# hebench/reference-seal-backend

Hardware: AMD Instinct MI355X
Metric: ciphertext-ops/sec (CKKS ct x ct mul+relin+rescale, N=2^15, L=16) (higher is better)
Workload: dtype u64 (exact residues; fp64-FMA engine for primes < 2^47, u64 Harvey engine with the fold reduction for the 60-bit primes)

## Files before the change

### reference-seal-backend_amd/csrc/device_tables.h

```cpp
#pragma once
#include <cstring>
#include <vector>

#include "he_params.h"
#include "client/multiword.h"

namespace he355 {

inline void prime_dev_fill(PrimeDev &d, const PrimeTables &pt, size_t N)
{
    const ArU64 au = pt.aru();
    const ArF64 af = pt.arf();
    d.q = pt.q; d.cr0 = pt.mod.cr0; d.cr1 = pt.mod.cr1;
    d.ninv = au.ninv; d.ninv_q = au.ninv_q;
    d.qd = af.q; d.qinv = af.qinv; d.ninv_d = af.ninv; d.ninv_i = af.ninv_i;
    d.fwd = nullptr; d.inv = nullptr; d.inv_w0_scaled = pt.inv_w0_scaled;
    d.f64 = pt.f64 ? 1 : 0;
    d.acc_terms = pt.f64 ? floor_direct_terms(pt.q) : 0;
    for (size_t k = 0; k < 64; ++k) d.colw[k] = 0.0;
    if (pt.f64)
        for (size_t k = 0; k < 32 && k < N; ++k) { d.colw[k] = ArF64::tw_w(pt.fwd[k]); d.colw[32 + k] = ArF64::tw_w(pt.inv[k]); }
    d.k2_direct = d.k2_lift = 0;
    d.pow32 = (double)((((u64)1) << 32) % pt.q);
}

enum K2Class { kK2General = 0, kK2Direct = 1, kK2Lift = 2 };
inline K2Class k2_lift_class(u64 qj, u64 qt, int logn1)
{
    const bool df = (qj >> 52) == 0, direct = df && !(qj > 2 * qt);
    double m = df ? (direct ? (double)qj : 0.5 * (double)qt + 1.0) : (double)qt;
    for (int st = 0; st < logn1; ++st) m += (double)qt * (0.5 + m * 4.440892098500626e-16);
    if (!(m * 1.0000001 < 140737488355328.0)) return kK2General;
    return direct ? kK2Direct : kK2Lift;
}
inline void k2_lift_masks(const Params &P, PrimeDev *pd)
{
    for (size_t j = 0; j < P.K; ++j)
        for (size_t t = 0; t < P.K; ++t) {
            if (!P.primes[t].f64) continue;
            const K2Class c = k2_lift_class(P.primes[j].q, P.primes[t].q, P.logn1);
            if (c == kK2General) continue;
            (c == kK2Direct ? pd[j].k2_direct : pd[j].k2_lift) |= (u64)1 << t;
        }
}

inline FloorConst floor_const(u64 qs, u64 qi, bool fold)
{
    FloorConst f;
    std::memset(&f, 0, sizeof(f));
    const u64 inv = Params::invmod(qs % qi, qi);
    f.inv = inv;
    f.inv_shoup = pre_word(inv, qi, fold);
    f.inv_d = (double)inv;
    f.inv_i = (double)inv / (double)qi;
    f.half_mod = (qs >> 1) % qi;
    f.src_mod = qs % qi;
    return f;
}
inline std::vector<FloorConst> floor_const_table(const Params &P)
{
    const size_t K = P.K;
    std::vector<FloorConst> fc(K * K);
    for (size_t s = 0; s < K; ++s)
        for (size_t i = 0; i < K; ++i)
            if (s != i) fc[s * K + i] = floor_const(P.primes[s].q, P.primes[i].q, P.primes[i].fold);
    return fc;
}

struct CrtTablesHost {
    int L = 0, words = 0;
    size_t o_half = 0, o_punct = 0, o_inv = 0;
    std::vector<u64> h;
    double Qd = 0;
};
inline CrtTablesHost crt_tables_host(const Params &P, int L)
{
    CrtTablesHost c;
    const int words = L + 2;
    c.L = L; c.words = words;
    c.o_half = words; c.o_punct = 2 * (size_t)words; c.o_inv = c.o_punct + (size_t)L * words;
    c.h.assign(c.o_inv + L, 0);
    u64 *Q = c.h.data(), *halfQ = Q + c.o_half;
    Q[0] = 1;
    for (int i = 0; i < L; ++i) client::mw_mul_small(Q, words, P.primes[i].q);
    for (int i = 0; i < words; ++i) halfQ[i] = (Q[i] >> 1) | (i + 1 < words ? Q[i + 1] << 63 : 0);
    for (int i = 0; i < L; ++i) {
        u64 *p = c.h.data() + c.o_punct + (size_t)i * words;
        p[0] = 1;
        u64 pm = 1;
        const u64 qi = P.primes[i].q;
        for (int k = 0; k < L; ++k)
            if (k != i) {
                client::mw_mul_small(p, words, P.primes[k].q);
                pm = (u64)(((u128)pm * (P.primes[k].q % qi)) % qi);
            }
        c.h[c.o_inv + i] = Params::invmod(pm, qi);
// ... 7 lines not shown
```

### reference-seal-backend_amd/csrc/he355_api.hip

```cpp
#include <hip/hip_runtime.h>

#include <array>
#include <algorithm>
#include <cerrno>
#include <cstdlib>
#include <cstdio>
#include <cstring>
#include <map>
#include <random>
#include <memory>
#include <stdexcept>
#include <string>
#include <vector>

#include "../../include/he355.h"
#include "behz_lists.h"
#include "bfv_pir_args.h"
#include "device_pool.h"
#include "device_tables.h"
#include "he355_internal.h"
#include "he355_kernels.h"
#include "he_params.h"
#include "hoist_args.h"
#include "ntt_core.h"
// ... 112 lines not shown
    const u64 r0 = __builtin_amdgcn_s_memrealtime(), c0 = __builtin_amdgcn_s_memtime();
    u64 r = r0;
    while (r - r0 < ticks_100mhz) {
        __builtin_amdgcn_s_sleep(127);
        r = __builtin_amdgcn_s_memrealtime();
    }
    const u64 c1 = __builtin_amdgcn_s_memtime();
    if (threadIdx.x == 0) { out[0] = c1 - c0; out[1] = r - r0; }
}

class DeviceContext {
public:
    DeviceContext(const Params &p, int device) : P(p), device_(device)
    {
        if (p.K + p.aux.size() + 1 > (size_t)kMaxPrimes) throw std::invalid_argument("too many primes for one device context (key chain + auxiliary primes exceed 64)");
        int count = 0;
        hipError_t e = hipGetDeviceCount(&count);
        if (e != hipSuccess || count <= 0) throw DeviceError("no HIP device available (the MI355X backend has no CPU fallback)");
        if (device < 0 || device >= count) throw DeviceError("invalid device ordinal");
        HIPCHECK(hipSetDevice(device));
        try {
            init();
        } catch (...) {
            teardown();
            throw;
        }
    }
    ~DeviceContext() { teardown(); }

private:
    void init()
    {
        HIPCHECK(hipStreamCreateWithFlags(&stream_, hipStreamNonBlocking));
        HIPCHECK(hipStreamCreateWithFlags(&stream2_, hipStreamNonBlocking));
        HIPCHECK(hipEventCreateWithFlags(&ev_fork_, hipEventDisableTiming));
        HIPCHECK(hipEventCreateWithFlags(&ev_join_, hipEventDisableTiming));
        HIPCHECK(hipEventCreate(&ev0_));
        HIPCHECK(hipEventCreate(&ev1_));
        const size_t N = P.N, K = P.K;
        const bool with_t = P.scheme == kSchemeBFV && P.plain_modulus > 2 && (P.plain_modulus - 1) % (2 * N) == 0;
        if (with_t) plain_tables_ = Params::make_prime_tables(P.plain_modulus, N, P.logn, true);
        t_index_ = with_t ? (int)(K + P.aux.size()) : -1;
        const size_t n_all = K + P.aux.size() + (with_t ? 1 : 0);
        std::vector<PrimeDev> pd(n_all);
        for (size_t i = 0; i < n_all; ++i) {
            const PrimeTables &pt = i < K ? P.primes[i] : i < K + P.aux.size() ? P.aux[i - K] : plain_tables_;
            Tw16 *dfwd = upload_owned(pt.fwd.data(), N), *dinv = upload_owned(pt.inv.data(), N);
            prime_dev_fill(pd[i], pt, N);
            pd[i].fwd = dfwd; pd[i].inv = dinv;
            env_.prime_f64[i] = pt.f64 ? 1 : 0;
            env_.prime_q[i] = pt.q;
        }
        k2_lift_masks(P, pd.data());
        d_primes_ = upload_owned(pd.data(), n_all);
        d_floor_ = upload_owned(floor_const_table(P).data(), K * K);
        env_.primes = d_primes_;
        env_.floor_consts = d_floor_;
        env_.N = (int)N; env_.logn1 = P.logn1; env_.K = (int)K; env_.Ltop = (int)P.Ltop; env_.scheme = P.scheme;
        env_.stream = stream_;
        env_.u64_fold = P.u64_fold;
        const char *ds = std::getenv("HE355_DUAL_STREAM");
        if (ds) dual_stream_ = ds[0] != '0';
        lim_.N = N; lim_.K = (int)K;
        u64 v = 0;
        if (env_u64("HE355_LATENCY_MAX", v)) set_latency_max(v);
        if (env_u64("HE355_LDS_MAX", v)) set_lds_max(v);
        if (env_u64("HE355_CHUNK", v) && v > 0) lim_.chunk = (size_t)v;
        int cus = 0;
        HIPCHECK(hipDeviceGetAttribute(&cus, hipDeviceAttributeMultiprocessorCount, device_));
        cus_ = cus > 0 ? (u64)cus : 1;
    }
    void teardown()
    {
        (void)hipSetDevice(device_);
        for (hipStream_t s : {stream_, stream2_, probe_stream_})
            if (s) (void)hipStreamSynchronize(s);
        for (void *p : owned_) pool_.raw_free(p);
        pool_.raw_free(d_relin_);
        pool_.raw_free(d_relin_scaled_);
        for (auto &kv : d_galois_) pool_.raw_free(kv.second);
        for (auto &kv : d_hoist_) pool_.raw_free(kv.second.p);
        for (Arena &a : arena_) pool_.raw_free(a.p);
        pool_.destroy();
        for (hipEvent_t e : {ev_fork_, ev_join_, ev0_, ev1_})
            if (e) (void)hipEventDestroy(e);
        for (hipStream_t s : {stream2_, probe_stream_, stream_})
            if (s) (void)hipStreamDestroy(s);
    }

public:
    void use() { HIPCHECK(hipSetDevice(device_)); }
    template <class T> void dmalloc(T *&p, size_t bytes) { p = static_cast<T *>(pool_.raw_malloc(bytes)); }
    template <class T> T *upload_owned(const T *h, size_t count)
    {
        T *d = nullptr;
        dmalloc(d, count * sizeof(T));
        owned_.push_back(d);
        if (h) HIPCHECK(hipMemcpy(d, h, count * sizeof(T), hipMemcpyHostToDevice));
        return d;
    }
    void *pool_alloc(size_t bytes)
    {
        use();
        return pool_.alloc(bytes);
    }
    void pool_free(void *p)
// ... 234 lines not shown
        KsBuffers ks;
        u64 *rlr;
        u64 *f;
    };
    enum { kScratch0, kScratch1,
           kLat0, kLat1,
           kRotTmp,
           kBfv,
           kClient,
           kGroups,
           kArenas };
    u64 *reserve(Arena &a, size_t bytes)
    {
        if (bytes <= a.bytes) return a.p;
        HIPCHECK(hipStreamSynchronize(stream_));
        HIPCHECK(hipStreamSynchronize(stream2_));
        pool_.raw_free(a.p);
        a = Arena{};
        dmalloc(a.p, bytes);
        a.bytes = bytes;
        return a.p;
    }
    bool try_reserve(Arena *first, int count, size_t need, bool last_resort = false)
    {
        size_t grow = 0, reclaim = pool_.cached_bytes();
        for (Arena *a = first; a != first + count; ++a)
            if (need > a->bytes) { grow += need; reclaim += a->bytes; }
        size_t free_b = 0, total_b = 0;
        if (grow && hipMemGetInfo(&free_b, &total_b) == hipSuccess && (double)grow > 0.9 * (double)(free_b + reclaim)) return false;
        try {
            for (Arena *a = first; a != first + count; ++a) reserve(*a, need);
            return true;
        } catch (const OutOfDeviceMemory &) {
            if (last_resort) throw;
            return false;
        }
    }
    size_t chunk_ops(u64 n, int L, bool may_dual)
    {
        const size_t per_op = scratch_words_per_op(P.N, L) * 8;
        const size_t c = halve_until_fit(std::min<u64>(lim_.chunk, n ? n : 1), [&](size_t k) { return try_reserve(&arena_[kScratch0], (may_dual && n > k) ? 2 : 1, per_op * k, k == 1); });
        if (!c) throw OutOfDeviceMemory("HIP error: out of device memory: the key-switch scratch of one ciphertext (" + std::to_string(per_op) + " bytes) does not fit");
        return c;
    }
    Scratch scratch(size_t c, int L, int which = 0)
    {
        const size_t N = P.N, LN = (size_t)L * N;
        const size_t per_op = scratch_words_per_op(N, L);
        Scratch s;
        u64 *p = reserve(arena_[kScratch0 + which], per_op * c * 8);
        s.ks.c01 = p; p += c * 2 * LN; s.ks.c01_item_stride = 2 * LN;
        s.ks.c2n = p; p += c * LN;
        s.ks.c2r = p; p += c * LN;
        s.ks.d = p; p += c * (size_t)(L + 1) * LN;
        s.ks.t = p; p += c * 2 * LN;
        s.ks.tp = p; p += c * 2 * N;
        s.ks.tpr = p; p += c * 2 * N;
        s.ks.e = p; p += c * 2 * LN;
        s.rlr = p; p += c * 3 * N;
        s.f = p;
        return s;
    }

    bool fuse_pays(const KernelEnv &e, u64 nc, int L) const { return he355::fuse_pays(ks_dims(e), nc, L); }
    bool level_sum_pays(const KernelEnv &e, int L, u64 n) const { return he355::level_sum_pays(ks_dims(e), lim_, L, n); }
    bool latency_shape(const KernelEnv &e, u64 nc) const { return he355::latency_shape(ks_dims(e), lim_, nc); }
    bool lds_shape(const KernelEnv &e, int L, u64 nc) const { return he355::lds_shape(ks_dims(e), lim_, L, nc); }
    KsShape ks_shape(const KernelEnv &e, int L, u64 nc, KsKind kind, bool out_apart) const { return he355::ks_shape(ks_dims(e), lim_, L, nc, kind, out_apart); }
    u64 *lds_part(const Scratch &S, int L) const
    {
        const size_t need = (size_t)ks_lds_part_words(env_, L), have = scratch_words_per_op(P.N, L) - 2 * (size_t)L * P.N;
        if (need > have) throw std::logic_error("ring-in-LDS key switch: the arena is too small for the partial products");
        return S.ks.c2n;
    }

    struct KsSource {
        KsKind kind;
        const u64 *a = nullptr, *b = nullptr;
        Indexer ix{};
        const u64 *addend = nullptr;
        uint32_t elt = 0;
        const uint32_t *table = nullptr;
        const u64 *key = nullptr;
        KsGroups groups{};
        bool coeff = false;
    };
    KernelEnv batch_env(int which = 0, bool ntt = false) const
    {
        KernelEnv env = env_;
        env.stream = which ? stream2_ : stream_;
        if (ntt) env.scheme = kSchemeCKKS;
        return env;
    }
    template <class F> void for_each_chunk(u64 n, int L, size_t chunk, bool may_dual, F &&f)
    {
        const bool dual = may_dual && n > chunk;
        u64 ci = 0;
        for (u64 off = 0; off < n; off += chunk, ++ci) {
            const int which = dual ? (int)(ci & 1) : 0;
            const bool fork = dual && ci == 0;
            f(off, std::min<u64>(chunk, n - off), which, scratch(std::min<u64>(chunk, n), L, which), fork ? ev_fork_ : nullptr);
            if (fork) HIPCHECK(hipStreamWaitEvent(stream2_, ev_fork_, 0));
        }
        if (dual) {
            HIPCHECK(hipEventRecord(ev_join_, stream2_));
            HIPCHECK(hipStreamWaitEvent(stream_, ev_join_, 0));
// ... 919 lines not shown
        float tot = 0;
        for (int i = 0; i < probe_.used; ++i) {
            float ms = 0;
            HIPCHECK(hipEventSynchronize(probe_.stop[i]));
            HIPCHECK(hipEventElapsedTime(&ms, probe_.start[i], probe_.stop[i]));
            tot += ms;
        }
        if (total_ms) *total_ms = tot;
        if (launches) *launches = (u64)probe_.used;
        if (ops) *ops = probe_.ops;
    }
    float timer_end()
    {
        use();
        HIPCHECK(hipEventRecord(ev1_, stream_));
        HIPCHECK(hipEventSynchronize(ev1_));
        float ms = 0;
        HIPCHECK(hipEventElapsedTime(&ms, ev0_, ev1_));
        env_.probe = nullptr;
        return ms;
    }
    void sync() { use(); HIPCHECK(hipStreamSynchronize(stream_)); HIPCHECK(hipStreamSynchronize(stream2_)); }
    void clock_probe_begin(u64 duration_us)
    {
        use();
        if (duration_us == 0 || duration_us > 10000000) throw std::invalid_argument("clock probe duration must be in (0, 10 s]");
        if (!probe_stream_) HIPCHECK(hipStreamCreateWithFlags(&probe_stream_, hipStreamNonBlocking));
        if (!d_clock_) d_clock_ = upload_owned<u64>(nullptr, 2);
        HIPCHECK(hipMemsetAsync(d_clock_, 0, 2 * sizeof(u64), probe_stream_));
        hipLaunchKernelGGL(k_clock_probe, dim3(1), dim3(64), 0, probe_stream_, duration_us * 100, d_clock_);
        HIPCHECK(hipGetLastError());
    }
    void clock_probe_end(double *mhz, double *seconds)
    {
        use();
        if (!probe_stream_ || !d_clock_) throw std::logic_error("clock probe not started");
        u64 h[2] = {0, 0};
        HIPCHECK(hipMemcpyAsync(h, d_clock_, sizeof h, hipMemcpyDeviceToHost, probe_stream_));
        HIPCHECK(hipStreamSynchronize(probe_stream_));
        if (mhz) *mhz = h[1] ? (double)h[0] / (double)h[1] * 100.0 : 0.0;
        if (seconds) *seconds = (double)h[1] / 1e8;
    }

private:
    KernelProbe probe_;
    const Params &P;
    int device_;
    hipStream_t stream_ = nullptr;
    hipEvent_t ev0_ = nullptr, ev1_ = nullptr;
    KernelEnv env_{};
    PrimeDev *d_primes_ = nullptr;
    KsLimits lim_;
    FloorConst *d_floor_ = nullptr;
    std::vector<void *> owned_;
    u64 *d_relin_ = nullptr;
    u64 *d_relin_scaled_ = nullptr;
    bool d_relin_scaled_ok_ = false;
    PrimeTables plain_tables_;
    int t_index_ = -1;
    EncTablesDev enc_{nullptr, nullptr, nullptr};
    int *d_err_ = nullptr;
    u64 *d_pk_ = nullptr, *d_sk_ = nullptr;
    u64 zero_seed_ = os_seed(), zero_index_ = 0;
    std::map<int, CrtTablesDev> crt_;
    std::map<int, BfvDeltaConst> bfv_delta_;
    std::map<int, BfvNoiseConst> bfv_noise_;
    BfvDropConst *d_bfv_drop_ = nullptr;
    std::map<uint32_t, u64 *> d_galois_;
    std::map<uint32_t, const uint32_t *> d_perm_, d_gather_;
    Arena arena_[kArenas];
    hipStream_t stream2_ = nullptr;
    hipStream_t probe_stream_ = nullptr;
    u64 *d_clock_ = nullptr;
    hipEvent_t ev_fork_ = nullptr, ev_join_ = nullptr;
    bool dual_stream_ = true;
    std::map<uint32_t, std::array<unsigned char, 32>> perm_rows_;
    Counters count_;
    struct HoistKey { u64 *p = nullptr; bool ok = false; };
    std::map<uint32_t, HoistKey> d_hoist_;
    u64 cus_ = 1;
    bool level_walk_ = !(getenv("HE355_LEVEL_WALK") && getenv("HE355_LEVEL_WALK")[0] == '0');
    size_t groups_next_ = 0;
    std::map<int, BehzDev> behz_;
    DevicePool pool_;
};

}

using namespace he355;

struct he355_ctx {
    std::unique_ptr<Params> params;
    std::unique_ptr<DeviceContext> dev;
};

static thread_local std::string g_last_error;

template <class F> static int guarded(F &&f)
{
    try {
        f();
        return HE355_OK;
    } catch (const DeviceError &e) {
        g_last_error = e.what();
        return HE355_E_DEVICE;
    } catch (const std::invalid_argument &e) {
// ... 477 lines not shown
```

### reference-seal-backend_amd/csrc/he355_kernels.h

```cpp
#pragma once
#include <hip/hip_runtime.h>

#include <cstdlib>
#include <utility>

#include "device_types.h"
#include "behz_core.h"
#include "bfv_level_core.h"
#include "bfv_noise_core.h"
#include "bfv_digits_core.h"
#include "bfv_bytes_core.h"
#include "bfv_reply_core.h"
#include "bfv_gadget_core.h"
#include "ks_shape.h"

namespace he355 {

struct KernelProbe {
    static constexpr int kCap = 2048;
    hipEvent_t start[kCap], stop[kCap];
    int created = 0, used = 0;
    u64 ops = 0;
};

struct KernelEnv {
    KernelProbe *probe = nullptr;
    const PrimeDev *primes;
    const FloorConst *floor_consts;
    int N, logn1, K, Ltop, scheme;
    hipStream_t stream;
    bool u64_fold = false;
    unsigned char prime_f64[kMaxPrimes];
    u64 prime_q[kMaxPrimes];
};




struct KsBuffers {
    u64 *c01;
    u64 c01_item_stride;
    u64 *c2n;
    u64 *c2r;
    u64 *d;
    u64 *t;
    u64 *tp;
    u64 *tpr;
    u64 *e;
};
struct KsGroups {
    const uint32_t *const *perm = nullptr;
    const u64 *const *key = nullptr;
    const u32 *src_block = nullptr;
    u32 group_size = 0;
    u64 *sum_out = nullptr;
    const u32 *count = nullptr;
};
constexpr u32 kGroupKeepBit = 0x80000000u;
constexpr int kMoveListCap = 64;
enum K1Mode { K1_MUL = 0, K1_CT3 = 1, K1_GALOIS = 2 };
struct K1Operands {
    K1Mode mode = K1_MUL;
    const u64 *a = nullptr, *b = nullptr;
    Indexer ix{};
    u64 op_offset = 0;
    const uint32_t *perm = nullptr;
    const u64 *addend = nullptr;
    bool no_c01 = false;
    bool no_c1 = false;
    bool no_c0n = false;
    const KsGroups *groups = nullptr;
};
enum K3Part { K3_ALL = 0, K3_SPECIAL_ONLY = 1, K3_DATA_ONLY = 2 };
struct K3Fuse {
    const u64 *cols;
    u64 *c01;
    u64 c01_item_stride;
    int tt_lo, tt_hi;
    const u64 *cols2;
    u64 *out;
    u64 *raw_tail = nullptr;
    const u64 *ta = nullptr, *tb = nullptr;
    Indexer tix{};
    u64 t_op_offset = 0;
    int c1_mode = 0;
    const u64 *c1_src = nullptr;
    const u64 *gsrc = nullptr;
    const uint32_t *gperm = nullptr;
    u64 gsrc_op_offset = 0;
};
inline KsDims ks_dims(const KernelEnv &env) { return KsDims{env.scheme, env.logn1, env.K}; }
inline bool k3_can_fuse(const KernelEnv &env) { return k3_can_fuse(ks_dims(env)); }
struct FloorRowsArgs {
    int src_prime, n_tgt, n_src;
    const u64 *cols;
    const u64 *tsrc; u64 tsrc_op_stride, tsrc_poly_stride;
// ... 147 lines not shown
```

### reference-seal-backend_amd/csrc/he355_kernels.hip

```cpp
#include <hip/hip_runtime.h>

#include <cstdio>
#include <cstdlib>
#include <stdexcept>
#include <type_traits>

#include "he355_kernels.h"
#include "ntt_core.h"
#include "client/ckks_codec.h"
#include "client/multiword.h"
#include "client/sampler.h"

#if !defined(HE355_KNS) || !defined(HE355_U64_FOLD)
#error "he355_kernels.hip is compiled once per form of the u64 engine: -DHE355_KNS=ks_shoup -DHE355_U64_FOLD=0 and -DHE355_KNS=ks_fold -DHE355_U64_FOLD=1 (Makefile)"
#endif
namespace he355 {
namespace HE355_KNS {
namespace {

#include "kernel_common.inc"

template <class Ar>
__device__ __forceinline__ void rows_fwd_job(const PrimeDev &P, u64 *row, bool in_raw, u32 rowbase, int lane, u64 *lds, bool valid)
{
// ... 336 lines not shown
    if (P.f64) mul3_acc_pair(make_ar(P, (ArF64 *)nullptr), P.q, pa, pb, a_stride_k * ct, b_stride_k * ct, P1, e2, inner, s0, s1, s2);
    else mul3_acc_pair(make_ar(P, (ArU64 *)nullptr), P.q, pa, pb, a_stride_k * ct, b_stride_k * ct, P1, e2, inner, s0, s1, s2);
    u64 *po = out + r * 3 * P1 + i * poly;
    reinterpret_cast<ulonglong2 *>(po)[e2] = s0;
    reinterpret_cast<ulonglong2 *>(po + P1)[e2] = s1;
    reinterpret_cast<ulonglong2 *>(po + 2 * P1)[e2] = s2;
}

template <class Ar, int BLOCK>
__device__ __forceinline__ typename std::conditional<std::is_same<Ar, ArF64>::value, TwRowF64, TwRow>::type
stage_row_twiddles(const PrimeDev &P, const Ar &ar, u32 rowbase, unsigned char *twl_raw, bool inverse = false)
{
    constexpr bool kF64 = std::is_same<Ar, ArF64>::value;
    typename std::conditional<kF64, TwRowF64, TwRow>::type twr;
    const gtw_t gf = gtw(inverse ? P.inv : P.fwd);
    constexpr int kIter = (kRowTw + BLOCK - 1) / BLOCK;
    Tw16 tmp[kIter];
#pragma unroll
    for (int k = 0; k < kIter; ++k) {
        const u32 i = threadIdx.x + k * BLOCK;
        tmp[k] = tw_load(gf, tw_row_source(rowbase, i + 1 < (u32)kRowTw ? i : 0));
    }
    if constexpr (kF64) {
        double *twl = reinterpret_cast<double *>(twl_raw);
#pragma unroll
        for (int k = 0; k < kIter; ++k)
            if (threadIdx.x + k * BLOCK < (u32)kRowTw) twl[threadIdx.x + k * BLOCK] = ArF64::tw_w(tmp[k]);
        twr.t = twl;
        twr.qinv = ar.qinv;
    } else {
        Tw16 *twl = reinterpret_cast<Tw16 *>(twl_raw);
#pragma unroll
        for (int k = 0; k < kIter; ++k)
            if (threadIdx.x + k * BLOCK < (u32)kRowTw) twl[threadIdx.x + k * BLOCK] = tmp[k];
        twr.t = twl;
    }
    return twr;
}

constexpr int K1_MUL_C2 = 3;
struct K1Args {
    const u64 *addend;
    const u64 *a, *b;
    Indexer ix;
    const uint32_t *perm;
    u64 *c01; u64 c01_item_stride;
    u64 *c2n, *c2r;
    u64 n_ops, op_offset;
    int L, logn1, mode;
    int no_c1;
    int no_c0n;
    int n_i;
    unsigned char i_list[64];
    KsGroups groups;
};

struct K1RowsC2 {
    u64 a1[kRowE], b1[kRowE];
};
__device__ __forceinline__ void k1_load_rows_c2(const K1Args &A, u64 op, int i, u32 a_row, int lane, K1RowsC2 &R)
{
    const u64 N = (u64)(1u << A.logn1) << kRowLog, P1 = (u64)A.L * N;
    const u64 roff = (u64)i * N + ((u64)a_row << kRowLog);
    const u64 r = A.op_offset + op;
    load_rowC(A.a + (idx_a(A.ix, r) * 2 + 1) * P1 + roff, lane, R.a1);
    load_rowC(A.b + (idx_b(A.ix, r) * 2 + 1) * P1 + roff, lane, R.b1);
}

template <class Ar, int MODE, class ITW = int>
__device__ __forceinline__ void k1_job(const K1Args &A, const PrimeDev &P, u64 op, int i, u32 a_row, int lane, u64 *lds, bool valid, const ITW *staged = nullptr,
                                       const K1RowsC2 *rows_c2 = nullptr)
{
    typedef typename Ar::T T;
    const Ar ar = make_ar(P, (Ar *)nullptr);
    const u32 n1 = 1u << A.logn1;
    const u64 N = (u64)n1 << kRowLog, P1 = (u64)A.L * N;
    const u64 roff = (u64)i * N + ((u64)a_row << kRowLog);
    u64 *c0p = A.c01 + op * A.c01_item_stride + roff;
    u64 *c1p = c0p + P1;
    u64 *c2np = A.c2n + op * P1 + roff;
    u64 *c2rp = A.c2r + op * P1 + roff;
    T x[kRowE];
    u64 v0[kRowE], v1[kRowE];
    if (MODE == K1_MUL || MODE == K1_MUL_C2) {
        const u64 r = A.op_offset + op;
        const u64 *pa = A.a + idx_a(A.ix, r) * 2 * P1 + roff, *pb = A.b + idx_b(A.ix, r) * 2 * P1 + roff;
        u64 a0[kRowE], a1[kRowE], b0[kRowE], b1[kRowE];
        u64 v2[kRowE];
        if (MODE == K1_MUL_C2) {
#pragma unroll
            for (int r2 = 0; r2 < kRowE; ++r2) x[r2] = ar.dy_mul(ar.dy_in(rows_c2->a1[r2]), ar.dy_in(rows_c2->b1[r2]));
        } else {
        load_rowC(pa, lane, a0); load_rowC(pa + P1, lane, a1);
        load_rowC(pb, lane, b0); load_rowC(pb + P1, lane, b1);
#pragma unroll
        for (int r2 = 0; r2 < kRowE; ++r2) {
            const T x0 = ar.dy_in(a0[r2]), x1 = ar.dy_in(a1[r2]), y0 = ar.dy_in(b0[r2]), y1 = ar.dy_in(b1[r2]);
            v0[r2] = ar.dy_out(ar.dy_mul(x0, y0));
            v1[r2] = ar.dy_out(ar.dy_add(ar.dy_mul(x0, y1), ar.dy_mul(x1, y0)));
            v2[r2] = ar.dy_out(ar.dy_mul(x1, y1));
            x[r2] = ar.from_canon(v2[r2]);
        }
        if (valid) { store_rowC(c0p, lane, v0); store_rowC(c1p, lane, v1); store_rowC(c2np, lane, v2); }
        }
    } else if (MODE == K1_CT3) {
        const u64 *pa = A.a + (A.op_offset + op) * 3 * P1 + roff;
// ... 10 lines not shown
        const uint32_t *perm = A.perm;
        if (A.groups.group_size) {
            const u32 gop = (u32)(A.op_offset + op), grp = gop / A.groups.group_size;
            src_ct = (u64)A.groups.src_block[grp] * A.groups.group_size + gop % A.groups.group_size;
            perm = A.groups.perm[grp];
        }
        const u64 *p0 = A.a + src_ct * 2 * P1 + (u64)i * N;
        const uint32_t *pm = perm + ((u64)a_row << kRowLog);
        u64 v2[kRowE];
        {
            const u64 *srow = p0 + (u64)(__builtin_amdgcn_readfirstlane(pm[0]) & ~(u32)(kRowN - 1));
            u32 pl[kRowE];
#pragma unroll
            for (int r2 = 0; r2 < kRowE; ++r2) pl[r2] = lds_pad((int)(pm[elemC(lane, r2)] & (u32)(kRowN - 1)));
            u64 t[kRowE];
            load_rowC(srow + P1, lane, t);
            lds_store_C(lds, lane, t);
            HE_WAVE_SYNC();
#pragma unroll
            for (int r2 = 0; r2 < kRowE; ++r2) v2[r2] = lds[pl[r2]];
            if (!A.no_c0n) {
                load_rowC(srow, lane, t);
                HE_WAVE_SYNC();
                lds_store_C(lds, lane, t);
                HE_WAVE_SYNC();
#pragma unroll
                for (int r2 = 0; r2 < kRowE; ++r2) v0[r2] = lds[pl[r2]];
            }
            HE_WAVE_SYNC();
#pragma unroll
            for (int r2 = 0; r2 < kRowE; ++r2) {
                if (A.no_c0n) v0[r2] = 0;
                v1[r2] = 0;
                x[r2] = ar.from_canon(v2[r2]);
            }
        }
        if (A.addend && !A.no_c0n) {
            const u64 *ad = A.addend + (A.op_offset + op) * 2 * P1 + roff;
            u64 a0[kRowE];
            load_rowC(ad, lane, a0);
            if (!A.no_c1) load_rowC(ad + P1, lane, v1);
#pragma unroll
            for (int r2 = 0; r2 < kRowE; ++r2) v0[r2] = addmod(v0[r2], a0[r2], P.q);
        }
        if (valid) {
            if (!A.no_c0n) store_rowC(c0p, lane, v0);
            if (!A.no_c1) store_rowC(c1p, lane, v1);
            store_rowC(c2np, lane, v2);
        }
    }
    const bool last = A.logn1 == 0;
    if constexpr (std::is_same<ITW, int>::value) wave_rows_inv(ar, P, last, n1 + a_row, lane, lds, x);
    else wave_rows_inv_tw(ar, *staged, P.inv_w0_scaled, last, lane, lds, x);
#pragma unroll
    for (int r2 = 0; r2 < kRowE; ++r2) v0[r2] = last ? ar.to_canon(x[r2]) : ar.to_raw(x[r2]);
    if (valid) store_rowA(c2rp, lane, v0);
}

template <int MODE, class Ar>
__global__ void __launch_bounds__(kBlock) k_k1(K1Args A, const PrimeDev *primes)
{
    __shared__ u64 lds[kWaves][kLdsRow];
    constexpr bool kF64 = std::is_same<Ar, ArF64>::value;
    __shared__ __attribute__((aligned(16))) unsigned char twl_raw[kF64 ? kRowTw * 8 : kRowTw * 16];
    const int wave = threadIdx.x >> 6, lane = threadIdx.x & 63;
    const u32 n1 = 1u << A.logn1;
    const u64 n_opg = (A.n_ops + kWaves - 1) / kWaves;
    const u64 tile = blockIdx.x / n_opg, opg = blockIdx.x % n_opg;
    const u32 a_row = (u32)(tile & (n1 - 1));
    const int i = A.i_list[tile >> A.logn1];
    u64 op = opg * kWaves + wave;
    const bool valid = op < A.n_ops;
    if (!valid) op = A.n_ops - 1;
    const PrimeDev &P = primes[i];
    const Ar ar = make_ar(P, (Ar *)nullptr);
    if constexpr (MODE == K1_MUL_C2) {
        K1RowsC2 rows;
        k1_load_rows_c2(A, op, i, a_row, lane, rows);
        const auto itw = stage_row_twiddles<Ar, kBlock>(P, ar, n1 + a_row, twl_raw, true);
        __syncthreads();
        k1_job<Ar, MODE>(A, P, op, i, a_row, lane, lds[wave], valid, &itw, &rows);
    } else {
        const auto itw = stage_row_twiddles<Ar, kBlock>(P, ar, n1 + a_row, twl_raw, true);
        __syncthreads();
        k1_job<Ar, MODE>(A, P, op, i, a_row, lane, lds[wave], valid, &itw);
    }
}
template <int MODE, class Ar>
__device__ __forceinline__ void k1_block(const K1Args &A, const PrimeDev *primes, const unsigned bid_x, u64 (*lds)[kLdsRow])
{
    const int wave = threadIdx.x >> 6, lane = threadIdx.x & 63;
    const u32 n1 = 1u << A.logn1;
    const u64 total = A.n_ops * A.n_i * n1;
    u64 job = (u64)bid_x * kWaves + wave;
    const bool valid = job < total;
    if (!valid) job = total - 1;
    const u32 a_row = (u32)(job & (n1 - 1));
    const u64 oi = job >> A.logn1;
    const int i = A.i_list[oi % A.n_i];
    const u64 op = oi / A.n_i;
    k1_job<Ar, MODE>(A, primes[i], op, i, a_row, lane, lds[wave], valid);
}
template <int MODE>
__global__ void __launch_bounds__(kBlock) k_k1_dual(K1Args AF, K1Args AU, unsigned n_f, const PrimeDev *primes)
{
    __shared__ u64 lds[kWaves][kLdsRow];
    if (blockIdx.x < n_f) k1_block<MODE, ArF64>(AF, primes, blockIdx.x, lds);
    else k1_block<MODE, ArU64>(AU, primes, blockIdx.x - n_f, lds);
}

struct K2Args {
    const u64 *c2r;
    u64 src_op_stride;
    u64 *d;
    u64 n_ops;
    int L, K, ckks, src_is_coeff;
    u64 f64_mask;
    int n_dig;
    unsigned char dig_list[64];
    int tsplit;
};

__device__ __forceinline__ double lift_wide(const ArF64 &ar, u64 v, double pow32)
{
    return ar.mulmod_vv((double)(u32)(v >> 32), pow32) + (double)(u32)v;
}
typedef const __attribute__((address_space(4))) double *cdw_t;
__device__ __forceinline__ cdw_t cdw(const double *p) { return (cdw_t)(unsigned long long)p; }
typedef u32 u32x2_t __attribute__((ext_vector_type(2)));
constexpr u32 kSlotBytes = kRowN * 8;
__device__ __forceinline__ __amdgpu_buffer_rsrc_t poly_rsrc(const void *p, u32 bytes)
{
    const unsigned long long v = (unsigned long long)p;
    const u32 lo = __builtin_amdgcn_readfirstlane((u32)v), hi = __builtin_amdgcn_readfirstlane((u32)(v >> 32));
    return __builtin_amdgcn_make_buffer_rsrc((void *)(((unsigned long long)hi << 32) | lo), 0, (int)bytes, 0x00020000);
}
template <int N1> __device__ __forceinline__ void store_pattern_rows(__amdgpu_buffer_rsrc_t dst, u32 off4, u32 off2h, const double x[N1])
{
#pragma unroll
    for (int a = 0; a < N1; ++a) {
        union { u64 u; double d; } c;
        c.d = x[a];
        __builtin_amdgcn_raw_buffer_store_b32((u32)c.u, dst, (int)off4, a * (int)kSlotBytes, 0);
        __builtin_amdgcn_raw_buffer_store_b16((unsigned short)(c.u >> 32), dst, (int)off2h, a * (int)kSlotBytes, 0);
    }
}
template <int N1> __device__ __forceinline__ void store_word_rows(__amdgpu_buffer_rsrc_t dst, u32 off8, const u64 x[N1])
{
#pragma unroll
    for (int a = 0; a < N1; ++a) {
        u32x2_t v;
        v.x = (u32)x[a]; v.y = (u32)(x[a] >> 32);
        __builtin_amdgcn_raw_buffer_store_b64(v, dst, (int)off8, a * (int)kSlotBytes, 0);
    }
}
typedef u32 u32x4_t __attribute__((ext_vector_type(4)));
template <int N1>
__device__ __forceinline__ void store_pattern_rows_wide(__amdgpu_buffer_rsrc_t dst, unsigned char *tile, int lane, u32 lane_lo, u32 lane_hi, const double x[N1])
{
    static_assert(N1 % 8 == 0, "written for whole groups of 8 rows");
    u32 *lo = reinterpret_cast<u32 *>(tile);
    unsigned short *hi = reinterpret_cast<unsigned short *>(tile + N1 * 256);
#pragma unroll
    for (int a = 0; a < N1; ++a) {
        union { u64 u; double d; } c;
// ... 1182 lines not shown
    if (!n_cts || !n_groups) return;
    const int logN = env.logn1 + kRowLog;
    const u64 threads = (n_cts * 2 * L) << (logN - 1);
    hipLaunchKernelGGL(k_sum_groups, dim3(grid_for(threads, kBlock)), dim3(kBlock), 0, env.stream, in, out, d_mult, env.primes, L, 2 * L, logN, n_cts, n_groups);
}

void launch_move_cts(const KernelEnv &env, u64 *dst, const u64 *src, const uint32_t *idx, u64 n, u64 elems_per_ct, bool scatter)
{
    const u64 pairs = elems_per_ct / 2;
    for (u64 off = 0; off < n; off += kMoveListCap) {
        const u64 m = std::min<u64>(kMoveListCap, n - off);
        MoveList list;
        for (u64 g = 0; g < m; ++g) list.idx[g] = idx[off + g];
        hipLaunchKernelGGL(k_move_cts, dim3(grid_for(pairs, kBlock), (unsigned)m), dim3(kBlock), 0, env.stream, scatter ? dst : dst + off * elems_per_ct,
                           scatter ? src + off * elems_per_ct : src, list, pairs, scatter ? 1 : 0);
    }
}

void launch_mul3_acc(const KernelEnv &env, int L, u64 rows, u64 cols, int inner, const u64 *a, u64 a_stride_i, u64 a_stride_k, const u64 *b,
                     u64 b_stride_k, u64 b_stride_j, u64 *out)
{
    const int logN = env.logn1 + kRowLog;
    const u64 threads = (rows * cols * (u64)L) << (logN - 1);
    hipLaunchKernelGGL(k_mul3_acc, dim3(grid_for(threads, kBlock)), dim3(kBlock), 0, env.stream, a, b, out, env.primes, L, logN, rows, cols, inner,
                       a_stride_i, a_stride_k, b_stride_k, b_stride_j);
}

void launch_mul3(const KernelEnv &env, int L, u64 n_results, const u64 *a, const u64 *b, Indexer ix, u64 *out)
{
    if (!n_results) return;
    const int logN = env.logn1 + kRowLog;
    const u64 threads = (n_results * L) << (logN - 1);
    hipLaunchKernelGGL(k_mul3, dim3(grid_for(threads, kBlock)), dim3(kBlock), 0, env.stream, a, b, out, ix, env.primes, L, logN, n_results);
}

constexpr unsigned kDualMaxBlocksK3 = 4096, kDualMaxBlocks = 1024;
void launch_k1(const KernelEnv &env, int L, u64 n_ops, const K1Operands &src, const KsBuffers &buf)
{
    if (!n_ops) return;
    const K1Mode mode = src.mode;
    const u64 *const addend = src.addend;
    const KsGroups *const groups = src.groups;
    const bool no_c01 = src.no_c01, no_c1 = src.no_c1, no_c0n = src.no_c0n;
    if (groups && (mode != K1_GALOIS || addend)) throw std::runtime_error("grouped launch: rotations without addend only");
    if (no_c01 && mode != K1_MUL) throw std::runtime_error("no_c01: the ct x ct multiply only");
    if (no_c1 && mode != K1_GALOIS && mode != K1_CT3) throw std::runtime_error("no_c1: rotations and size-3 inputs only");
    K1Args A;
    A.no_c1 = no_c1 ? 1 : 0;
    if (no_c0n && (mode != K1_GALOIS || !no_c1 || (addend && groups))) throw std::runtime_error("no_c0n: rotations whose polynomial 1 is left to k_k3 only");
    A.no_c0n = no_c0n ? 1 : 0;
    A.groups = groups ? *groups : KsGroups{};
    A.a = src.a; A.b = src.b; A.ix = src.ix; A.perm = src.perm; A.addend = addend;
    A.c01 = buf.c01; A.c01_item_stride = buf.c01_item_stride; A.c2n = buf.c2n; A.c2r = buf.c2r;
    A.n_ops = n_ops; A.op_offset = src.op_offset; A.L = L; A.logn1 = env.logn1; A.mode = (int)mode;
    K1Args AP[2];
    unsigned gp[2] = {0, 0};
    for (int pass = 0; pass < 2; ++pass) {
        A.n_i = 0;
        for (int i = 0; i < L; ++i)
            if ((env.prime_f64[i] != 0) == (pass == 0)) A.i_list[A.n_i++] = (unsigned char)i;
        AP[pass] = A;
        gp[pass] = A.n_i ? grid_for((n_ops * A.n_i) << env.logn1, kWaves) : 0;
    }
    const hipStream_t st = env.stream;
    if (gp[0] && gp[1] && (n_ops <= 8 || gp[0] + gp[1] <= kDualMaxBlocks) && mode != K1_MUL_C2 && !(mode == K1_MUL && no_c01)) {
        const dim3 grid(gp[0] + gp[1]);
        if (mode == K1_MUL) hipLaunchKernelGGL((k_k1_dual<K1_MUL>), grid, dim3(kBlock), 0, st, AP[0], AP[1], gp[0], env.primes);
        else if (mode == K1_CT3) hipLaunchKernelGGL((k_k1_dual<K1_CT3>), grid, dim3(kBlock), 0, st, AP[0], AP[1], gp[0], env.primes);
        else hipLaunchKernelGGL((k_k1_dual<K1_GALOIS>), grid, dim3(kBlock), 0, st, AP[0], AP[1], gp[0], env.primes);
        return;
    }
    for (int pass = 0; pass < 2; ++pass) {
        if (!gp[pass]) continue;
        const K1Args &AA = AP[pass];
        const dim3 grid((unsigned)((((u64)AA.n_i) << env.logn1) * ((n_ops + kWaves - 1) / kWaves)));
        if (pass == 0) {
            if (mode == K1_MUL && no_c01) hipLaunchKernelGGL((k_k1<K1_MUL_C2, ArF64>), grid, dim3(kBlock), 0, st, AA, env.primes);
            else if (mode == K1_MUL) hipLaunchKernelGGL((k_k1<K1_MUL, ArF64>), grid, dim3(kBlock), 0, st, AA, env.primes);
            else if (mode == K1_CT3) hipLaunchKernelGGL((k_k1<K1_CT3, ArF64>), grid, dim3(kBlock), 0, st, AA, env.primes);
            else hipLaunchKernelGGL((k_k1<K1_GALOIS, ArF64>), grid, dim3(kBlock), 0, st, AA, env.primes);
        } else {
            if (mode == K1_MUL && no_c01) hipLaunchKernelGGL((k_k1<K1_MUL_C2, ArU64>), grid, dim3(kBlock), 0, st, AA, env.primes);
            else if (mode == K1_MUL) hipLaunchKernelGGL((k_k1<K1_MUL, ArU64>), grid, dim3(kBlock), 0, st, AA, env.primes);
            else if (mode == K1_CT3) hipLaunchKernelGGL((k_k1<K1_CT3, ArU64>), grid, dim3(kBlock), 0, st, AA, env.primes);
            else hipLaunchKernelGGL((k_k1<K1_GALOIS, ArU64>), grid, dim3(kBlock), 0, st, AA, env.primes);
        }
    }
}

void launch_k2(const KernelEnv &env, int L, u64 n_ops, const KsBuffers &buf, const u64 *src, u64 src_op_stride, int tsplit)
{
    if (!n_ops) return;
    K2Args A;
    A.c2r = src ? src : buf.c2r;
    A.src_op_stride = src ? src_op_stride : (u64)L * env.N;
    A.src_is_coeff = src ? 1 : 0;
    A.d = buf.d; A.n_ops = n_ops; A.L = L; A.K = env.K; A.ckks = env.scheme == 2;
    A.f64_mask = 0; A.tsplit = tsplit > 1 ? tsplit : 1;
    for (int t = 0; t < env.K; ++t) A.f64_mask |= (u64)(env.prime_f64[t] != 0) << t;
    auto target_split = [&](unsigned gw) {
        if (tsplit > 1) return tsplit;
        int ts = 1;
        const int n_tgt = L + 1 - (A.ckks ? 1 : 0);
        auto cost = [&](int c) { return (double)(((u64)gw * c + 511) / 512) * (1.0 + 1.2 * ((n_tgt + c - 1) / c)); };
        const double c1 = cost(1);
        double best = c1;
        for (int c = 2; c <= 4; c <<= 1)
            if (cost(c) < best * 0.95 && cost(c) < c1 * 0.95) { best = cost(c); ts = c; }
        return ts;
    };
    K2Args AK[2];
    unsigned gk[2] = {0, 0};
    for (int wide = 0; wide < 2; ++wide) {
        A.n_dig = 0;
        for (int j = 0; j < L; ++j)
            if ((env.prime_q[j] >> 52 != 0) == (wide != 0)) A.dig_list[A.n_dig++] = (unsigned char)j;
        AK[wide] = A;
        gk[wide] = (unsigned)(n_ops * A.n_dig * 4);
    }
    if (gk[0] && gk[1]) {
        const int ts = target_split(gk[0] + gk[1]);
        if (tsplit > 1 || (gk[0] + gk[1]) * (unsigned)ts <= kDualMaxBlocks) {
            AK[0].tsplit = AK[1].tsplit = ts;
            const dim3 gd(gk[0] + gk[1], (unsigned)ts);
#define HE355_K2D(L1) case L1: hipLaunchKernelGGL((k_k2n_dual<L1>), gd, dim3(kBlock), 0, env.stream, AK[0], AK[1], gk[0], env.primes); break;
            switch (env.logn1) { HE355_K2D(0) HE355_K2D(1) HE355_K2D(2) HE355_K2D(3) HE355_K2D(4) HE355_K2D(5) }
#undef HE355_K2D
            return;
        }
    }
    for (int wide = 0; wide < 2; ++wide) {
        if (!gk[wide]) continue;
        AK[wide].tsplit = target_split(gk[wide]);
        const dim3 gd(gk[wide], (unsigned)AK[wide].tsplit);
#define HE355_K2N(L1)                                                                                                         \
    case L1:                                                                                                                  \
        if (wide) hipLaunchKernelGGL((k_k2n<L1, true>), gd, dim3(kBlock), 0, env.stream, AK[wide], env.primes);               \
        else hipLaunchKernelGGL((k_k2n<L1, false>), gd, dim3(kBlock), 0, env.stream, AK[wide], env.primes);                   \
        break;
        switch (env.logn1) { HE355_K2N(0) HE355_K2N(1) HE355_K2N(2) HE355_K2N(3) HE355_K2N(4) HE355_K2N(5) }
#undef HE355_K2N
    }
}


void launch_k3(const KernelEnv &env, int L, u64 n_ops, const KsBuffers &buf, const u64 *key, K3Part part, const K3Fuse *fuse, int n_split, u64 *split_part,
               int n_split_u64, const KsGroups *groups, u64 g_op_offset)
// ... 473 lines not shown
```

### reference-seal-backend_amd/csrc/k2n_body.inc

```
    constexpr int N1 = 1 << LOGN1;
    constexpr u64 N = (u64)N1 << kRowLog;
    const u64 oj = K2N_BID_X >> 2;
    const u32 cb = K2N_BID_X & 3;
    const int col = (int)(cb << 8) | threadIdx.x;
    const u32 oj32 = (u32)oj;
    const int j = A.dig_list[__builtin_amdgcn_readfirstlane(oj32 % (u32)A.n_dig)];
    const u64 op = __builtin_amdgcn_readfirstlane(oj32 / (u32)A.n_dig);
    const u64 *src = A.c2r + op * A.src_op_stride + (u64)j * N;
    const PrimeDev &Pj = primes[j];
    const bool coeff_in = A.src_is_coeff || LOGN1 == 0;
    constexpr bool kTile = N1 >= 8;
    __shared__ __attribute__((aligned(16))) unsigned char tiles[kTile ? kWaves : 1][kTile ? N1 * 384 : 16];
    unsigned char *tile = tiles[kTile ? threadIdx.x >> 6 : 0];
    if constexpr (WIDE) {
        u64 c[N1];
        if (coeff_in) {
#pragma unroll
            for (int a = 0; a < N1; ++a) c[a] = src[(a << kRowLog) + col];
        } else {
            const ArU64 ar = make_ar(Pj, (ArU64 *)nullptr);
            u64 x[N1];
#pragma unroll
            for (int a = 0; a < N1; ++a) x[a] = src[(a << kRowLog) + col];
            col_inv<ArU64, LOGN1>(ar, x, ctw(Pj.inv), Pj.inv_w0_scaled);
#pragma unroll
            for (int a = 0; a < N1; ++a) c[a] = ar.to_canon(x[a]);
        }
        k2n_targets_f64<LOGN1, false>(A, primes, Pj, j, op, c, col, tile);
        k2n_targets_u64<LOGN1>(A, primes, Pj, j, op, c, col);
    } else {
    double c[N1];
    if (coeff_in) {
#pragma unroll
        for (int a = 0; a < N1; ++a) c[a] = u52_to_f64(src[(a << kRowLog) + col]);
    } else if (Pj.f64) {
        const ArF64 ar = make_ar(Pj, (ArF64 *)nullptr);
#pragma unroll
        for (int a = 0; a < N1; ++a) c[a] = ar.from_raw(src[(a << kRowLog) + col]);
        col_inv<ArF64, LOGN1>(ar, c, ctw(Pj.inv), Pj.inv_w0_scaled);
#pragma unroll
        for (int a = 0; a < N1; ++a) c[a] = ar.canon(c[a]);
    } else {
        const ArU64 ar = make_ar(Pj, (ArU64 *)nullptr);
        u64 x[N1];
#pragma unroll
        for (int a = 0; a < N1; ++a) x[a] = src[(a << kRowLog) + col];
        col_inv<ArU64, LOGN1>(ar, x, ctw(Pj.inv), Pj.inv_w0_scaled);
#pragma unroll
        for (int a = 0; a < N1; ++a) c[a] = u52_to_f64(ar.to_canon(x[a]));
    }
    k2n_targets_f64<LOGN1, true>(A, primes, Pj, j, op, c, col, tile);
    u64 cu[N1];
#pragma unroll
    for (int a = 0; a < N1; ++a) cu[a] = f64_to_u52(c[a]);
    k2n_targets_u64<LOGN1>(A, primes, Pj, j, op, cu, col);
    }
```

### reference-seal-backend_amd/csrc/kernel_common.inc

```
constexpr int kBlock = 256;
constexpr int kWaves = 4;

#define HE_WAVE_SYNC()                                             \
    do {                                                           \
        __builtin_amdgcn_fence(__ATOMIC_RELEASE, "wavefront");     \
        __builtin_amdgcn_wave_barrier();                           \
        __builtin_amdgcn_fence(__ATOMIC_ACQUIRE, "wavefront");     \
    } while (0)

__device__ __forceinline__ gtw_t gtw(const Tw16 *p) { return (gtw_t)p; }
__device__ __forceinline__ ctw_t ctw(const Tw16 *p) { return (ctw_t)(unsigned long long)p; }

__device__ __forceinline__ ArU64 make_ar(const PrimeDev &p, ArU64 *)
{
    ArU64 a;
    a.q = p.q; a.two_q = p.q * 2; a.ninv = p.ninv; a.ninv_q = p.ninv_q; a.cr0 = p.cr0; a.cr1 = p.cr1;
    return a;
}
__device__ __forceinline__ ArF64 make_ar(const PrimeDev &p, ArF64 *)
{
    ArF64 a;
    a.q = p.qd; a.qinv = p.qinv; a.ninv = p.ninv_d; a.ninv_i = p.ninv_i;
    return a;
}
// ... 42 lines not shown
    case 1: launch(std::integral_constant<int, 1>()); break;
    case 2: launch(std::integral_constant<int, 2>()); break;
    case 3: launch(std::integral_constant<int, 3>()); break;
    case 4: launch(std::integral_constant<int, 4>()); break;
    case 5: launch(std::integral_constant<int, 5>()); break;
    default: throw std::invalid_argument("ring size out of range");
    }
}
template <class What>
unsigned grid_blocks(u64 blocks, What what, const char *unit = "polynomials")
{
    if (blocks > 0x7fffffffull) throw std::invalid_argument(std::string(what) + ": too many " + unit + " for one launch");
    return (unsigned)blocks;
}
template <class What>
unsigned streaming_grid(u64 n_polys, int logN, What what, const char *unit = "polynomials")
{
    return grid_blocks((n_polys << (logN - 1)) / kBlock, what, unit);
}

constexpr int kMacG = 4;

typedef __attribute__((address_space(3))) void lds_void_t;
template <int PIECES = 8>
__device__ __forceinline__ void dma_row_to_lds(const u64 *grow, u64 *lds_row, int lane)
{
    const u32 lbase = __builtin_amdgcn_readfirstlane((u32)(unsigned long long)(lds_void_t *)lds_row);
    const u64 *g = grow + (lane << 1);
#pragma unroll
    for (int k = 0; k < PIECES; ++k)
        asm volatile("s_mov_b32 m0, %0\n\ts_nop 0\n\tglobal_load_lds_dwordx4 %1, off nt" ::"s"(lbase + (u32)(k << 10)), "v"(g + (k << 7)) : "memory");
}
__device__ __forceinline__ void lds_rowA(const u64 *lds_row, int lane, u64 v[kRowE])
{
#pragma unroll
    for (int r = 0; r < kRowE; ++r) v[r] = lds_row[(r << 6) | lane];
}

constexpr double kPackBias = 4503599627370496.0 + 2251799813685248.0 + 140737488355328.0;
constexpr int kPackHiOff = 4096;
__device__ __forceinline__ double unpack48(u32 lo, u32 hi16)
{
    union { u64 u; double d; } c;
    c.u = ((u64)(0x43380000u | hi16) << 32) | lo;
    return c.d - kPackBias;
}
__device__ __forceinline__ void lds_rowA48(const u64 *lds_row, int lane, double x[kRowE])
{
    const u32 *lo = reinterpret_cast<const u32 *>(lds_row);
    const unsigned short *hi = reinterpret_cast<const unsigned short *>(reinterpret_cast<const unsigned char *>(lds_row) + kPackHiOff);
#pragma unroll
    for (int r = 0; r < kRowE; ++r) x[r] = unpack48(lo[(r << 6) | lane], hi[(r << 6) | lane]);
}
struct NoHook {
    __device__ __forceinline__ void operator()() const {}
};
template <class Ar, class TW, class Hook = NoHook, bool LAZY = false>
__device__ __forceinline__ void wave_rows_fwd_n(const Ar &ar, const TW &tw, int lane, u64 *lds_w, typename Ar::T (*x)[kRowE], Hook before_c = Hook())
{
    typedef typename Ar::T T;
    T *lds = reinterpret_cast<T *>(lds_w);
    Tw16 wa[kTwA];
    gather_A(tw, wa);
    if constexpr (LAZY) row_fwd_A_lazy<1>(ar, x, wa); else row_fwd_A<1>(ar, x, wa);
    Tw16 wb[kTwB];
    gather_B(tw, lane, wb);
    __builtin_amdgcn_sched_barrier(0);
    lds_store_A(lds, lane, x[0]);
    HE_WAVE_SYNC();
    lds_load_B(lds, lane, x[0]);
    HE_WAVE_SYNC();
    if constexpr (LAZY) row_fwd_B_lazy<1>(ar, x, wb); else row_fwd_B<1>(ar, x, wb);
    Tw16 wc[kTwC];
    gather_C(tw, lane, wc);
    before_c();
    __builtin_amdgcn_sched_barrier(0);
    lds_store_B(lds, lane, x[0]);
    HE_WAVE_SYNC();
    lds_load_C(lds, lane, x[0]);
    HE_WAVE_SYNC();
    if constexpr (LAZY) row_fwd_C_lazy<1>(ar, x, wc); else row_fwd_C<1>(ar, x, wc);
}
template <class Ar, class TW>
__device__ __forceinline__ void wave_rows_fwd(const Ar &ar, const TW &tw, int lane, u64 *lds_w, typename Ar::T x[kRowE])
{
    wave_rows_fwd_n(ar, tw, lane, lds_w, reinterpret_cast<typename Ar::T(*)[kRowE]>(x));
}
template <class Ar, class TW>
__device__ __forceinline__ void wave_rows_inv_tw(const Ar &ar, const TW &itw, const Tw16 &w0_scaled, bool last, int lane, u64 *lds_w, typename Ar::T x[kRowE])
{
    typedef typename Ar::T T;
    T *lds = reinterpret_cast<T *>(lds_w);
    row_inv_C(ar, x, itw, lane);
    Tw16 wb[kTwInvB];
    gather_inv_B(itw, lane, wb);
    __builtin_amdgcn_sched_barrier(0);
    lds_store_C(lds, lane, x);
    HE_WAVE_SYNC();
    lds_load_B(lds, lane, x);
    HE_WAVE_SYNC();
    row_inv_B_w(ar, x, wb);
    Tw16 wa[kTwInvA];
    gather_inv_A(itw, wa);
    __builtin_amdgcn_sched_barrier(0);
    lds_store_B(lds, lane, x);
    HE_WAVE_SYNC();
// ... 32 lines not shown
```

Before: 23520.

## Pack c2r intermediate rows as 48-bit values for fp64 primes in key-switch

For fp64-engine primes whose row-stage value bound provably stays below 2^47, the first key-switch kernel now writes the c2r intermediate as biased 48-bit packed values (a 32-bit low half and a 16-bit high half) instead of full u64 words. The consumer kernel unpacks them directly into doubles. The goal is to cut global memory traffic for this scratch buffer by about a quarter. The cost is a host-side bound analysis per prime, extra renormalization before packing, and reliance on the bound being correct. The packed layout's index strides in the consumer also have to match the producer's row layout.

```diff
diff --git a/reference-seal-backend_amd/csrc/device_tables.h b/reference-seal-backend_amd/csrc/device_tables.h
--- a/reference-seal-backend_amd/csrc/device_tables.h
+++ b/reference-seal-backend_amd/csrc/device_tables.h
@@ -42,6 +42,33 @@
             if (c == kK2General) continue;
             (c == kK2Direct ? pd[j].k2_direct : pd[j].k2_lift) |= (u64)1 << t;
         }
+}
+
+constexpr double kPack48Limit = 140737488355328.0;
+constexpr double kPack48Eps = 4.440892098500626e-16;
+constexpr int kC2rRecentred = 2;
+inline double c2r_row_bound(u64 q)
+{
+    const double qd = (double)q;
+    double b[16], top = 0.5 * qd + 1.0;
+    for (double &v : b) v = 0.5 * qd + 1.0;
+    for (int bit = 1; bit < 16; bit <<= 1)
+        for (int r = 0; r < 16; ++r) {
+            if (r & bit) continue;
+            const double s = b[r] + b[r | bit];
+            b[r] = s;
+            b[r | bit] = qd * (0.5 + s * kPack48Eps);
+        }
+    for (int r = kC2rRecentred; r < 16; ++r) top = b[r] > top ? b[r] : top;
+    return top;
+}
+inline bool c2r_packs(u64 q, int logn1) { return logn1 > 0 && (q >> 47) == 0 && c2r_row_bound(q) * 1.0000001 < kPack48Limit; }
+inline u64 c2r_pack_mask(const Params &P)
+{
+    u64 mask = 0;
+    for (size_t j = 0; j < P.K; ++j)
+        if (P.primes[j].f64 && c2r_packs(P.primes[j].q, P.logn1)) mask |= (u64)1 << j;
+    return mask;
 }
 
 inline FloorConst floor_const(u64 qs, u64 qi, bool fold)
diff --git a/reference-seal-backend_amd/csrc/he355_api.hip b/reference-seal-backend_amd/csrc/he355_api.hip
--- a/reference-seal-backend_amd/csrc/he355_api.hip
+++ b/reference-seal-backend_amd/csrc/he355_api.hip
@@ -188,6 +188,7 @@
             env_.prime_q[i] = pt.q;
         }
         k2_lift_masks(P, pd.data());
+        c2r_pack_ = c2r_pack_mask(P);
         d_primes_ = upload_owned(pd.data(), n_all);
         d_floor_ = upload_owned(floor_const_table(P).data(), K * K);
         env_.primes = d_primes_;
@@ -528,6 +529,7 @@
         s.ks.c01 = p; p += c * 2 * LN; s.ks.c01_item_stride = 2 * LN;
         s.ks.c2n = p; p += c * LN;
         s.ks.c2r = p; p += c * LN;
+        s.ks.c2r_pack = c2r_pack_;
         s.ks.d = p; p += c * (size_t)(L + 1) * LN;
         s.ks.t = p; p += c * 2 * LN;
         s.ks.tp = p; p += c * 2 * N;
@@ -1553,6 +1555,7 @@
     PrimeDev *d_primes_ = nullptr;
     KsLimits lim_;
     FloorConst *d_floor_ = nullptr;
+    u64 c2r_pack_ = 0;
     std::vector<void *> owned_;
     u64 *d_relin_ = nullptr;
     u64 *d_relin_scaled_ = nullptr;
diff --git a/reference-seal-backend_amd/csrc/he355_kernels.h b/reference-seal-backend_amd/csrc/he355_kernels.h
--- a/reference-seal-backend_amd/csrc/he355_kernels.h
+++ b/reference-seal-backend_amd/csrc/he355_kernels.h
@@ -42,6 +42,7 @@
     u64 c01_item_stride;
     u64 *c2n;
     u64 *c2r;
+    u64 c2r_pack = 0;
     u64 *d;
     u64 *t;
     u64 *tp;
diff --git a/reference-seal-backend_amd/csrc/he355_kernels.hip b/reference-seal-backend_amd/csrc/he355_kernels.hip
--- a/reference-seal-backend_amd/csrc/he355_kernels.hip
+++ b/reference-seal-backend_amd/csrc/he355_kernels.hip
@@ -412,6 +412,7 @@
     int no_c0n;
     int n_i;
     unsigned char i_list[64];
+    u64 c2r_pack;
     KsGroups groups;
 };
 
@@ -528,6 +529,15 @@
     const bool last = A.logn1 == 0;
     if constexpr (std::is_same<ITW, int>::value) wave_rows_inv(ar, P, last, n1 + a_row, lane, lds, x);
     else wave_rows_inv_tw(ar, *staged, P.inv_w0_scaled, last, lane, lds, x);
+    if constexpr (std::is_same<Ar, ArF64>::value) {
+        if ((A.c2r_pack >> i) & 1) {
+            x[0] = ar.renorm(x[0]); x[1] = ar.renorm(x[1]);
+#pragma unroll
+            for (int r2 = 0; r2 < kRowE; ++r2) x[r2] += kPackBias;
+            if (valid) store_rowA48(c2rp, lane, x);
+            return;
+        }
+    }
 #pragma unroll
     for (int r2 = 0; r2 < kRowE; ++r2) v0[r2] = last ? ar.to_canon(x[r2]) : ar.to_raw(x[r2]);
     if (valid) store_rowA(c2rp, lane, v0);
@@ -587,6 +597,7 @@
 
 struct K2Args {
     const u64 *c2r;
+    u64 c2r_pack;
     u64 src_op_stride;
     u64 *d;
     u64 n_ops;
@@ -1875,6 +1886,7 @@
     A.groups = groups ? *groups : KsGroups{};
     A.a = src.a; A.b = src.b; A.ix = src.ix; A.perm = src.perm; A.addend = addend;
     A.c01 = buf.c01; A.c01_item_stride = buf.c01_item_stride; A.c2n = buf.c2n; A.c2r = buf.c2r;
+    A.c2r_pack = env.logn1 > 0 ? buf.c2r_pack : 0;
     A.n_ops = n_ops; A.op_offset = src.op_offset; A.L = L; A.logn1 = env.logn1; A.mode = (int)mode;
     K1Args AP[2];
     unsigned gp[2] = {0, 0};
@@ -1916,6 +1928,7 @@
     if (!n_ops) return;
     K2Args A;
     A.c2r = src ? src : buf.c2r;
+    A.c2r_pack = src || env.logn1 == 0 ? 0 : buf.c2r_pack;
     A.src_op_stride = src ? src_op_stride : (u64)L * env.N;
     A.src_is_coeff = src ? 1 : 0;
     A.d = buf.d; A.n_ops = n_ops; A.L = L; A.K = env.K; A.ckks = env.scheme == 2;
diff --git a/reference-seal-backend_amd/csrc/k2n_body.inc b/reference-seal-backend_amd/csrc/k2n_body.inc
--- a/reference-seal-backend_amd/csrc/k2n_body.inc
+++ b/reference-seal-backend_amd/csrc/k2n_body.inc
@@ -35,8 +35,15 @@
         for (int a = 0; a < N1; ++a) c[a] = u52_to_f64(src[(a << kRowLog) + col]);
     } else if (Pj.f64) {
         const ArF64 ar = make_ar(Pj, (ArF64 *)nullptr);
+        if ((A.c2r_pack >> j) & 1) {
+            const u32 *lo = reinterpret_cast<const u32 *>(src);
+            const unsigned short *hi = reinterpret_cast<const unsigned short *>(reinterpret_cast<const unsigned char *>(src) + kPackHiOff);
 #pragma unroll
-        for (int a = 0; a < N1; ++a) c[a] = ar.from_raw(src[(a << kRowLog) + col]);
+            for (int a = 0; a < N1; ++a) c[a] = unpack48(lo[(a << (kRowLog + 1)) + col], hi[(a << (kRowLog + 2)) + col]);
+        } else {
+#pragma unroll
+            for (int a = 0; a < N1; ++a) c[a] = ar.from_raw(src[(a << kRowLog) + col]);
+        }
         col_inv<ArF64, LOGN1>(ar, c, ctw(Pj.inv), Pj.inv_w0_scaled);
 #pragma unroll
         for (int a = 0; a < N1; ++a) c[a] = ar.canon(c[a]);
diff --git a/reference-seal-backend_amd/csrc/kernel_common.inc b/reference-seal-backend_amd/csrc/kernel_common.inc
--- a/reference-seal-backend_amd/csrc/kernel_common.inc
+++ b/reference-seal-backend_amd/csrc/kernel_common.inc
@@ -118,6 +118,18 @@
 #pragma unroll
     for (int r = 0; r < kRowE; ++r) x[r] = unpack48(lo[(r << 6) | lane], hi[(r << 6) | lane]);
 }
+__device__ __forceinline__ void store_rowA48(u64 *row, int lane, const double x[kRowE])
+{
+    u32 *lo = reinterpret_cast<u32 *>(row);
+    unsigned short *hi = reinterpret_cast<unsigned short *>(reinterpret_cast<unsigned char *>(row) + kPackHiOff);
+#pragma unroll
+    for (int r = 0; r < kRowE; ++r) {
+        union { u64 u; double d; } c;
+        c.d = x[r];
+        lo[(r << 6) | lane] = (u32)c.u;
+        hi[(r << 6) | lane] = (unsigned short)(c.u >> 32);
+    }
+}
 struct NoHook {
     __device__ __forceinline__ void operator()() const {}
 };
```

Measured after the change: 23600, median of 6. No clear change (+0.4%).
